# his0si/ConvNet-Quantization

Measured on AMD Instinct MI355X. Metric: images/sec at batch 1024 (3×32×32) int8 static-PTQ, 1/2/4/8 MI355X; top-1 delta, higher is better.
Workload: dtype int8; 1 GPU; full static-PTQ SimpleConvNet, all conv+linear int8 (u8 x s8 -> i32), NHWC, per-tensor weights; global_batch=1024, per_gpu_batch=1024, parallelism=dp1

## Files before the change

convnet-quantization_amd/csrc/conv3x3.hip:

```cpp
#include "common.hpp"
#include "conv_epi.hpp"
#include <type_traits>
#include <utility>
#include <algorithm>
#include <cmath>
#include "qconvnet_abi.hpp"

namespace qcn {

constexpr int kPipeD = 2;
constexpr int kSm56D = 4;
constexpr int kProdPrio = 2;

template <int CIN, int COUT, int HW, bool POOL, int WPX, int PSP = 16, int RPAD = 0,
          int SPAD = 0, bool SPLIT = false, int WI_ = 2, int JT_ = 4, int RB_ = 0>
struct ConvCfg {
  static constexpr int kCin = CIN, kCout = COUT;
  static constexpr bool kPool = POOL, kSplit = SPLIT;
  static constexpr int W = HW, H = HW;
  static constexpr int WI = WI_;
  static constexpr int JT = JT_;
  static constexpr int MPS = JT * WI;
  static constexpr int kWpx = WPX;
  static constexpr int WCO = COUT / (32 * WI);
// ... 1259 lines not shown
  static constexpr int OFF_CA = OFF_EB + 12 * CB::kCout;
  static constexpr int OFF_CB = OFF_CA + 4 * CA::kCout;
  static constexpr int LDS = OFF_CB + 4 * CB::kCout;
  static_assert(LDS <= 160 * 1024, "LDS budget");
  static constexpr int OPI = CB::OPX / SEGS;
};

template <class CA, class CB, int FA, int FB, bool KMAJOR, bool ILV = false>
QCN_DEV void convpair_ws16_body(int b, int G, const uint8_t* __restrict__ x, int nimg, int x_zp,
                                const int8_t* __restrict__ wa, const ConvEpi& epa, int xb_zp,
                                const int8_t* __restrict__ wb, const ConvEpi& epb, uint8_t* __restrict__ y) {
  using P = PairWs16<CA, CB>;
  using XA = Pix16<CA>;
  using XB = Pix16<CB>;
  constexpr int SEGS = P::SEGS, IMG = CA::IMG, W = CA::W, WCO = CA::WCO;
  constexpr int CH16 = CA::kCin / 16;
  extern __shared__ __attribute__((aligned(16))) uint8_t lds[];
  const int tid = threadIdx.x;
  const int role = __builtin_amdgcn_readfirstlane(tid >> 8);
  const int rt = tid & 255, lane = tid & 63, wave = rt >> 6;
  const int wc = wave % WCO, wp = wave / WCO;
  int T;
  if constexpr (ILV) {
    const int mine = b < nimg ? (nimg - 1 - b) / G + 1 : 0;
    T = (mine + SEGS - 1) / SEGS;
  } else {
    const int ntile = (nimg + SEGS - 1) / SEGS;
    T = b < ntile ? (ntile - 1 - b) / G + 1 : 0;
  }
  auto img_of = [&](int k, int sg) {
    const int n = ILV ? b + (k * SEGS + sg) * G : (b + k * G) * SEGS + sg;
    return n < nimg ? n : (ILV ? b + k * SEGS * G : (b + k * G) * SEGS);
  };
  auto in_src = [&](int k, int q) {
    const int p = rt + 256 * q;
    const int n = img_of(k, p / (IMG * CH16));
    return x + ((long)n * IMG + (p / CH16) % IMG) * CA::kCin + (p % CH16) * 16;
  };
  auto in_dst = [&](int q) {
    const int p = rt + 256 * q;
    const int pix = (p / CH16) % IMG;
    return CA::slot(p / (IMG * CH16), pix / W + 1, pix % W + 1) + (p % CH16) * 16;
  };
  uint4 sv0[4];
  if (role == 0 && T > 0) {
#pragma unroll
    for (int q = 0; q < 4; ++q) sv0[q] = *reinterpret_cast<const uint4*>(in_src(0, q));
  }
  float* eka = reinterpret_cast<float*>(lds + P::OFF_EA);
  float* ekb = reinterpret_cast<float*>(lds + P::OFF_EB);
  int* cra = reinterpret_cast<int*>(lds + P::OFF_CA);
  int* crb = reinterpret_cast<int*>(lds + P::OFF_CB);
  constexpr int NA = 3 * CA::kCout / 4, NB = 3 * CB::kCout / 4;
  constexpr int NCA = CA::kCout / 4, NCB = CB::kCout / 4;
  constexpr int NTAB = NA + NB + NCA + NCB, TPT = (NTAB + 255) / 256;
  float4 tval[TPT];
  auto tab = [&](int e, bool dst) -> float4* {
    if (e < NA) {
      const int a = e / (CA::kCout / 4), o = e % (CA::kCout / 4);
      const float* s = a == 0 ? epa.u : (a == 1 ? epa.v : epa.mult);
      return dst ? reinterpret_cast<float4*>(eka) + e : const_cast<float4*>(reinterpret_cast<const float4*>(s) + o);
    }
    e -= NA;
    if (e < NB) {
      const int a = e / (CB::kCout / 4), o = e % (CB::kCout / 4);
      const float* s = a == 0 ? epb.u : (a == 1 ? epb.v : epb.mult);
      return dst ? reinterpret_cast<float4*>(ekb) + e : const_cast<float4*>(reinterpret_cast<const float4*>(s) + o);
    }
    e -= NB;
    if (e < NCA)
      return dst ? reinterpret_cast<float4*>(cra) + e
                 : const_cast<float4*>(reinterpret_cast<const float4*>(epa.corr) + e);
    e -= NCA;
    return dst ? reinterpret_cast<float4*>(crb) + e
               : const_cast<float4*>(reinterpret_cast<const float4*>(epb.corr) + e);
  };
  {
    const uint32_t pa4 = xor80(splat_u8(x_zp)), pb4 = xor80(splat_u8(xb_zp));
    auto halo = [&](auto cfg, uint8_t* base, int nbuf, int pbytes, uint32_t pad) {
      using C = decltype(cfg);
      constexpr int HS = 2 * C::PCOLS + 2 * (C::PROWS - 2), CH = C::kCin / 16;
      const int total = nbuf * C::SEGS * HS * CH;
      for (int e = tid; e < total; e += 512) {
        const int c = e % CH, hs = (e / CH) % HS, sg = (e / (CH * HS)) % C::SEGS, bf = e / (CH * HS * C::SEGS);
        int pr, pc;
        if (hs < C::PCOLS) { pr = 0; pc = hs; }
        else if (hs < 2 * C::PCOLS) { pr = C::PROWS - 1; pc = hs - C::PCOLS; }
        else { const int r = hs - 2 * C::PCOLS; pr = 1 + (r >> 1); pc = (r & 1) ? C::PCOLS - 1 : 0; }
        *reinterpret_cast<uint4*>(base + bf * pbytes + C::slot(sg, pr, pc) + c * 16) = make_uint4(pad, pad, pad, pad);
      }
    };
    halo(CA{}, lds + P::OFF_PA, P::DOUBLE_A ? 2 : 1, P::PA, pa4);
    halo(CB{}, lds + P::OFF_PB, 2, P::PB, pb4);
  }
  if (role == 1) {
#pragma unroll
    for (int k = 0; k < TPT; ++k)
      if (rt + 256 * k < NTAB) tval[k] = *tab(rt + 256 * k, false);
#pragma unroll
    for (int k = 0; k < TPT; ++k)
      if (rt + 256 * k < NTAB) *tab(rt + 256 * k, true) = tval[k];
  }
  if (T == 0) return;

  const int p16 = lane & 15, g = lane >> 4;
  const wt_rsrc_t wra = wt_rsrc(wa), wrb = wt_rsrc(wb);
  const int voff = (wc * 64 + p16) * 64 + g * 16;
  auto pa_buf = [&](int j) { return lds + P::OFF_PA + (P::DOUBLE_A ? (j & 1) * P::PA : 0); };
  auto pb_buf = [&](int j) { return lds + P::OFF_PB + (j & 1) * P::PB; };
  auto write_in = [&](uint8_t* pa, const uint4 (&sv)[4]) {
#pragma unroll
    for (int q = 0; q < 4; ++q)
      *reinterpret_cast<uint4*>(pa + in_dst(q)) =
          make_uint4(xor80(sv[q].x), xor80(sv[q].y), xor80(sv[q].z), xor80(sv[q].w));
  };
  auto first_chunk = [&](wt_rsrc_t w0, v4i (&ga)[2][4]) {
#pragma unroll
    for (int i = 0; i < 4; ++i) {
      const auto v = __builtin_amdgcn_raw_buffer_load_b128(w0, voff, i * 1024, 0);
      ga[0][i] = (v4i){(int)v[0], (int)v[1], (int)v[2], (int)v[3]};
    }
  };

  v4i acc[4][8];
  if (role == 0) write_in(pa_buf(0), sv0);
  lds_barrier();

  struct Lane {
    int p16, g, ek;
    int la, lb;
    int hb;
    int q;
    const int *ca, *cb;
  };
  auto lanes = [&]() {
    int lz = lane;
    asm volatile("" : "+v"(lz));
    Lane L;
    L.p16 = lz & 15;
    L.g = lz >> 4;
    L.ek = wc * 64 + 4 * L.g;
    L.la = XA::at(wp, 0, L.p16) + 16 * L.g;
    L.lb = XB::at(wp, 0, L.p16) + 16 * L.g;
    L.hb = XA::template out_at<CB>(wp, 0, L.p16) + wc * 64 + 4 * L.g;
    L.q = wp * 32 + L.p16;
    L.ca = cra + (lz >> 6);
    L.cb = crb + (lz >> 6);
    return L;
  };
  auto epi_a = [&](const Lane& L, uint8_t* pb) {
    static_for<4>([&](auto ic) {
      constexpr int i = decltype(ic)::value;
      const EpiG K = load_epig(eka, CA::kCout, L.ek + 16 * i);
      static_for<8>([&](auto jc) {
        constexpr int j = decltype(jc)::value;
        uint32_t wd = 0;
#pragma unroll
        for (int r = 0; r < 4; ++r) wd = rq_elem<FA>(acc[i][j][r], K, r, epa, wd);
        *reinterpret_cast<uint32_t*>(pb + L.hb + XA::template out_jofs<CB>(j) + 16 * i) = xor80(wd);
      });
    });
  };
  auto epi_b = [&](const Lane& L, int k) {
    static_for<2>([&](auto gc) {
      constexpr int gq = decltype(gc)::value;
      uint32_t d[4];
      static_for<4>([&](auto ic) {
        constexpr int i = decltype(ic)::value;
        const EpiG K = load_epig(ekb, CB::kCout, L.ek + 16 * i);
        uint32_t wd = 0;
#pragma unroll
        for (int r = 0; r < 4; ++r) {
          const int a = max(max(acc[i][4 * gq][r], acc[i][4 * gq + 1][r]),
                            max(acc[i][4 * gq + 2][r], acc[i][4 * gq + 3][r]));
          wd = rq_elem<FB>(a, K, r, epb, wd);
        }
        d[i] = wd;
      });
      const auto s02 = __builtin_amdgcn_permlane32_swap(d[0], d[2], false, false);
      const auto s13 = __builtin_amdgcn_permlane32_swap(d[1], d[3], false, false);
      const auto t01 = __builtin_amdgcn_permlane16_swap(s02[0], s13[0], false, false);
      const auto t23 = __builtin_amdgcn_permlane16_swap(s02[1], s13[1], false, false);
      const uint4 v = make_uint4(t01[0], t01[1], t23[0], t23[1]);
      const int q = L.q + 16 * gq;
      const int n = img_of(k, q / P::OPI), pix = q % P::OPI;
      const int co = wc * 64 + 16 * L.g;
      const bool real = ILV ? b + (k * SEGS + q / P::OPI) * G < nimg : (b + k * G) * SEGS + q / P::OPI < nimg;
      if (real) {
        if constexpr (KMAJOR) {
          const int kc = (pix * CB::kCout + co) / 32;
          store_wt16(wt_rsrc(y), (uint32_t)(((long)kc * nimg + n) * 32 + 16 * (L.g & 1)), v);
        } else {
          store_wt16(wt_rsrc(y + (long)n * P::OPI * CB::kCout), (uint32_t)(pix * CB::kCout + co), v);
        }
      }
    });
  };

  if (role == 0) {
    v4i ga[2][4];
    first_chunk(wra, ga);
    uint4 sv[4] = {};
#pragma unroll 1
    for (int p = 0; p <= T; ++p) {
      if constexpr (!P::DOUBLE_A) {
        if (p >= 1 && p < T) write_in(pa_buf(p), sv);
        lds_barrier();
      }
      WS16_STAMP(p, 0);
      if (p < T) {
        const Lane L = lanes();
        pipe_job16<CA>(pa_buf(p), L.ca, wra, wra, voff, wc, L.la, L.g, acc, ga);
        WS16_STAMP(p, 1);
        const int kn = p + 1 < T ? p + 1 : p;
#pragma unroll
        for (int q = 0; q < 4; ++q) sv[q] = *reinterpret_cast<const uint4*>(in_src(kn, q));
        epi_a(L, pb_buf(p));
        if constexpr (P::DOUBLE_A) write_in(pa_buf(p + 1), sv);
        WS16_STAMP(p, 2);
      }
      lds_barrier();
    }
  } else {
    v4i ga[2][4];
    first_chunk(wrb, ga);
#pragma unroll 1
    for (int p = 0; p <= T; ++p) {
      if constexpr (!P::DOUBLE_A) lds_barrier();
      WS16_STAMP(p, 0);
      if (p >= 1) {
        const Lane L = lanes();
        if (p >= 2) epi_b(L, p - 2);
        WS16_STAMP(p, 1);
        pipe_job16<CB>(pb_buf(p - 1), L.cb, wrb, wrb, voff, wc, L.lb, L.g, acc, ga);
        WS16_STAMP(p, 2);
      }
      lds_barrier();
    }
    const Lane L = lanes();
    epi_b(L, T - 1);
#ifdef QCN_CONVNET_STAMP
    if (T + 1 < 8) { WS16_STAMP(T + 1, 0); }
#endif
  }
}

template <class CA, class CB, int FA, int FB, bool KMAJOR>
__global__ __launch_bounds__(512, 1)
void convpair_ws16_kernel(const uint8_t* __restrict__ x, int nimg, int x_zp, const int8_t* __restrict__ wa,
                          ConvEpi epa, int xb_zp, const int8_t* __restrict__ wb, ConvEpi epb,
                          uint8_t* __restrict__ y) {
  convpair_ws16_body<CA, CB, FA, FB, KMAJOR>((int)blockIdx.x, (int)gridDim.x, x, nimg, x_zp, wa, epa, xb_zp,
                                             wb, epb, y);
}

using W16A3 = ConvCfg<64, 128, 16, false, 2, 32, 0, 0, false>;
using W16B4 = ConvCfg<128, 128, 16, true, 2, 32, 64, 0, true>;
using W16A5 = ConvCfg<128, 256, 8, false, 1, 32, 192, 0, false>;
using W16B6 = ConvCfg<256, 256, 8, true, 1, 32, 0, 0, true>;

struct Conv1Cfg {
  static constexpr int H = 32, W = 32, R = 16, COUT = 64, NT = 256;
  static constexpr int PXB = R * W;
  static constexpr int PR = R + 2, PC = W + 2;
  static constexpr int PATCH = 3 * PR * PC;
  static constexpr int PATCH_AL = (PATCH + 15) / 16 * 16;
  static constexpr int KS = 32 + 16;
  static constexpr int LDS = PATCH_AL + PXB * KS;
};

template <int HW>
__global__ __launch_bounds__(256, 3)
void conv1_f32_kernel(const float* __restrict__ x, int nimg, float in_inv, int in_zp,
                      const int8_t* __restrict__ w1, ConvEpi ep, uint8_t* __restrict__ y,
                      uint8_t* __restrict__ qin_out) {
  constexpr int H = HW, W = HW;
  constexpr int R = (HW * HW >= 512) ? 512 / W : H;
  constexpr int SEGS = (HW * HW >= 512) ? 1 : 512 / (HW * HW);
  constexpr int PR = R + 2, PC = W + 2;
  constexpr int PATCH = SEGS * 3 * PR * PC;
  constexpr int PATCH_AL = (PATCH + 15) / 16 * 16;
  constexpr int KS = 48;
  extern __shared__ __attribute__((aligned(16))) uint8_t lds[];
  int8_t* patch = reinterpret_cast<int8_t*>(lds);
  uint8_t* cols = lds + PATCH_AL;

  const int tid = threadIdx.x, lane = tid & 63, wave = tid >> 6;
  const int l32 = lane & 31, hi = lane >> 5;
  const long p0 = (long)blockIdx.x * 512;
  const int n0 = (int)(p0 / (H * W));
  const int y0 = (int)((p0 % (H * W)) / W);
  const int8_t padv = (int8_t)(in_zp - 128);

  for (int it = tid; it < PATCH; it += 256) {
    const int seg = it / (3 * PR * PC);
    const int rem = it % (3 * PR * PC);
    const int c = rem / (PR * PC);
    const int rr = (rem / PC) % PR, cc = rem % PC;
    const int n = n0 + seg, yy = y0 + rr - 1, xx = cc - 1;
    int8_t v = padv;
    if (n < nimg && yy >= 0 && yy < H && xx >= 0 && xx < W) {
      const long gi = (((long)n * 3 + c) * H + yy) * W + xx;
      float t = x[gi] * in_inv;
      t = fminf(fmaxf(t, -1.0e9f), 1.0e9f);
      int q = (int)__builtin_rintf(t) + in_zp;
      q = q < 0 ? 0 : (q > 255 ? 255 : q);
      v = (int8_t)(q - 128);
      if (qin_out != nullptr && seg < SEGS && rr >= 1 && rr <= R && cc >= 1 && cc <= W)
        qin_out[(((long)n * H + yy) * W + xx) * 3 + c] = (uint8_t)q;
    }
    patch[it] = v;
  }
  __syncthreads();
  for (int pp = tid; pp < 512; pp += 256) {
    const int seg = pp / (R * W), yy = (pp / W) % R, xx = pp % W;
    uint32_t wds[8];
#pragma unroll
    for (int d = 0; d < 8; ++d) {
      uint32_t wv = 0;
#pragma unroll
      for (int bb = 0; bb < 4; ++bb) {
        const int k = d * 4 + bb;
        uint32_t byte = 0;
        if (k < 27) {
          const int tap = k / 3, c = k % 3, r = tap / 3, s = tap % 3;
          byte = (uint8_t)patch[((seg * 3 + c) * PR + yy + r) * PC + xx + s];
        }
        wv |= byte << (8 * bb);
      }
      wds[d] = wv;
    }
    uint4* dst = reinterpret_cast<uint4*>(cols + pp * KS);
    dst[0] = make_uint4(wds[0], wds[1], wds[2], wds[3]);
    dst[1] = make_uint4(wds[4], wds[5], wds[6], wds[7]);
  }
  __syncthreads();

  v4i a[2];
#pragma unroll
  for (int i = 0; i < 2; ++i)
    a[i] = *reinterpret_cast<const v4i*>(w1 + (i * 32 + l32) * 32 + hi * 16);
  v16i acc[2][4];
#pragma unroll
  for (int j = 0; j < 4; ++j) {
    const int m = (wave * 4 + j) * 32 + l32;
    const v4i b = *reinterpret_cast<const v4i*>(cols + m * KS + hi * 16);
#pragma unroll
    for (int i = 0; i < 2; ++i)
      acc[i][j] = __builtin_amdgcn_mfma_i32_32x32x32_i8(a[i], b, acc_init_corr(ep.corr, i * 32, hi),
                                                        0, 0, 0);
  }
  __syncthreads();
  uint8_t* lout = lds;
#pragma unroll
  for (int i = 0; i < 2; ++i)
#pragma unroll
    for (int j = 0; j < 4; ++j)
      epilogue_tile<1>(&acc[i][j], ep, i * 32, hi, lout + ((wave * 4 + j) * 32 + l32) * 80);
  __syncthreads();
  const long total = (long)nimg * H * W;
  store_staged<64, 80, 256>(lout, 512, y + p0 * 64, total - p0, tid);
}

using Conv2Cfg = ConvCfg<64, 64, 32, true, 4, 16, 96, 0, true>;

struct Conv12P {
  using C = Conv2Cfg;
  static constexpr int PATCH = C::PATCH;
  static constexpr int WRES = 9 * C::WBUF;
  static constexpr int IN_R = 20, IN_C = 40;
  static constexpr int IN8 = IN_R * IN_C * 4;
  static constexpr int OFF_W = 2 * PATCH;
  static constexpr int OFF_IN = OFF_W + WRES;
  static constexpr int OFF_EPI1 = OFF_IN + 2 * IN8;
  static constexpr int OFF_EPI2 = OFF_EPI1 + 12 * 64;
  static constexpr int OFF_CORR2 = OFF_EPI2 + 12 * 64;
  static constexpr int OFF_A1 = OFF_CORR2 + 4 * 64;
  static constexpr int OFF_CORR1 = OFF_A1 + 2 * 64 * 16;
  static constexpr int LDS = OFF_CORR1 + 4 * 64;
  static_assert(LDS <= 160 * 1024, "LDS budget");
  static constexpr int OFF_QLUT = LDS;
  static constexpr int LDS_U8 = OFF_QLUT + 3 * 256;
  static_assert(OFF_QLUT % 4 == 0 && LDS_U8 <= 160 * 1024, "LDS budget");
};

template <class C>
QCN_DEV void conv_mainloop_res(const uint8_t* patch, const uint8_t* wres,
                               const int* __restrict__ corr, int wave, int lane,
                               v16i (&acc)[2][4]) {
  constexpr int CB = C::kCin / 64;
  const int wc = wave % C::WCO, wp = wave / C::WCO;
  const int l32 = lane & 31, hi = lane >> 5;
  const PatchAddr<C> pa(wp, l32, hi);
  const int arow = wc * 64 + l32;
  const int aswz = (arow >> 2) & 3;
  v16i c0[2];
#pragma unroll
  for (int i = 0; i < 2; ++i) c0[i] = acc_init_corr(corr, wc * 64 + i * 32, hi);
  const uint8_t* abase = wres + arow * 64;
  auto rd_a = [&](int ch, int kk, int i) {
    return *reinterpret_cast<const v4i*>(abase + ch * C::WBUF + i * 32 * 64 +
                                         (((2 * kk + hi) ^ aswz) << 4));
  };
  auto rd_b = [&](int ch, int kk, int j) {
    const int tap = ch / CB, cb = ch % CB;
    return *reinterpret_cast<const v4i*>(patch + pa.base[j] + PatchAddr<C>::delta(tap, j) + cb * 64 +
                                         kk * 32);
  };
  auto step = [&](v4i (&fan)[2], v4i (&fbn)[4], int rch, int rkk, bool rd,
                  const v4i (&fa)[2], const v4i (&fb)[4], bool first) {
#pragma unroll
    for (int m = 0; m < 8; ++m) {
      if (rd) {
        if (m < 2) fan[m] = rd_a(rch, rkk, m);
        else if (m < 6) fbn[m - 2] = rd_b(rch, rkk, m - 2);
      }
      __builtin_amdgcn_sched_barrier(0);
      acc[m >> 2][m & 3] = __builtin_amdgcn_mfma_i32_32x32x32_i8(
          fa[m >> 2], fb[m & 3], first ? c0[m >> 2] : acc[m >> 2][m & 3], 0, 0, 0);
      __builtin_amdgcn_sched_barrier(0);
    }
  };
  v4i fa0[2], fb0[4], fa1[2], fb1[4];
  fa0[0] = rd_a(0, 0, 0);
  fa0[1] = rd_a(0, 0, 1);
#pragma unroll
  for (int j = 0; j < 4; ++j) fb0[j] = rd_b(0, 0, j);
#pragma unroll
  for (int ch = 0; ch < C::NCH; ++ch) {
    step(fa1, fb1, ch, 1, true, fa0, fb0, ch == 0);
    step(fa0, fb0, ch + 1, 0, ch + 1 < C::NCH, fa1, fb1, false);
  }
}

#ifdef QCN_C12_STAMP
__device__ unsigned long long g_c12_stamp[4096][3][12][3];
QCN_DEV void c12_stamp(int j, int k) {
  const unsigned long long t = __builtin_amdgcn_s_memtime();
  const unsigned lane = __builtin_amdgcn_mbcnt_hi(~0u, __builtin_amdgcn_mbcnt_lo(~0u, 0u));
  const int w = threadIdx.x >> 6;
  const int s = w == 0 ? 0 : (w == 4 ? 1 : (w == 5 ? 2 : -1));
  if (s >= 0 && lane == 0 && blockIdx.x < 4096 && j < 12) {
    volatile unsigned long long* d = &g_c12_stamp[blockIdx.x][s][j][k];
    *d = t + lane;
  }
}
#define C12_STAMP(j, k) c12_stamp(j, k)
#else
#define C12_STAMP(j, k)
#endif

template <class XT>
QCN_DEV void conv12p_body(int t0, int ts, int T, const XT* __restrict__ x, int nimg,
                          float in_inv, int in_zp, const int8_t* __restrict__ w1, ConvEpi ep1,
                          int x2_zp, const int8_t* __restrict__ w2, ConvEpi ep2,
                          uint8_t* __restrict__ y, const uint8_t* __restrict__ qlut = nullptr) {
  using C = Conv2Cfg;
  using L = Conv12P;
  constexpr bool U8 = std::is_same<XT, uint8_t>::value;
  static_assert(U8 || std::is_same<XT, float>::value, "fp32 NCHW or u8 NHWC input");
  extern __shared__ __attribute__((aligned(16))) uint8_t lds[];
  const int tid = threadIdx.x, lane = tid & 63, wave = tid >> 6;
  const bool producer = wave >= 4;
  const int ptid = tid - 320;
  auto tile_of = [&](int j) { return (t0 + (j >> 1) * ts) * 2 + (j & 1); };
  uint8_t* patch0 = lds;
  uint8_t* patch1 = lds + L::PATCH;
  uint8_t* in8_0 = lds + L::OFF_IN;
  uint8_t* in8_1 = lds + L::OFF_IN + L::IN8;

  typename std::conditional<U8, uint32_t, float4>::type xraw[3];
  const uint32_t padw = xor80(splat_u8(x2_zp));
  const uint4 pad4 = make_uint4(padw, padw, padw, padw);
  for (int e = tid; e < 2 * C::PROWS * 8; e += 512) {
    const int buf = e / (C::PROWS * 8), r = e % (C::PROWS * 8);
    const int pr = r / 8, pc = ((r / 4) & 1) ? C::PCOLS - 1 : 0, chunk = r & 3;
    *reinterpret_cast<uint4*>(lds + buf * L::PATCH + C::slot(0, pr, pc) + chunk * 16) = pad4;
  }

  auto setup = [&]() {
    if (!producer) {
      const int wave_u = __builtin_amdgcn_readfirstlane(wave);
#pragma unroll
      for (int i = 0; i < L::WRES / 4096; ++i) {
        const int p = i * 4 + wave_u;
        const int o = p * 1024 + lane * 16;
        const int ch = o / C::WBUF, oc = o % C::WBUF;
        const int r = oc >> 6, sl = (oc >> 4) & 3;
        glds16(w2 + (long)ch * C::WBUF + r * 64 + ((sl ^ ((r >> 2) & 3)) << 4), lds + L::OFF_W + p * 1024);
      }
    }

    const uint32_t in_pad = xor80(splat_u8(in_zp)) & 0x00ffffffu;
    for (int e = tid; e < 2 * L::IN_R * L::IN_C; e += 512) {
      const int b = e / (L::IN_R * L::IN_C), rc = e % (L::IN_R * L::IN_C);
      const int rr = rc / L::IN_C, cc = rc % L::IN_C;
      const bool pad_row = b == 0 ? rr < 2 : rr >= 18;
      if (pad_row || cc < 4 || cc >= 36)
        reinterpret_cast<uint32_t*>(lds + L::OFF_IN + b * L::IN8)[rc] = in_pad;
    }
    if (!producer) stage_epik<64, 256>(ep1, reinterpret_cast<float*>(lds + L::OFF_EPI1), tid);
    if (!producer) stage_epik<64, 256>(ep2, reinterpret_cast<float*>(lds + L::OFF_EPI2), tid);
    {
      int t = tid;
      asm volatile("" : "+v"(t));
      if (t < 16)
        reinterpret_cast<int4*>(lds + L::OFF_CORR2)[t] = reinterpret_cast<const int4*>(ep2.corr)[t];
      if (t >= 64 && t < 80)
        reinterpret_cast<int4*>(lds + L::OFF_CORR1)[t - 64] = reinterpret_cast<const int4*>(ep1.corr)[t - 64];
    }
    if (wave == 3) {
      const int l32 = lane & 31, hi = lane >> 5;
      v4i* a1t = reinterpret_cast<v4i*>(lds + L::OFF_A1);
#pragma unroll
      for (int i = 0; i < 2; ++i) {
        const uint4 r0 = *reinterpret_cast<const uint4*>(w1 + (i * 32 + l32) * 32);
        const uint4 r1 = *reinterpret_cast<const uint4*>(w1 + (i * 32 + l32) * 32 + 16);
        const uint32_t wd[8] = {r0.x, r0.y, r0.z, r0.w, r1.x, r1.y, r1.z, r1.w};
        auto byte = [&](int k) -> uint32_t { return (wd[k >> 2] >> (8 * (k & 3))) & 0xff; };
        auto tapw = [&](int t) -> int {
          return (int)(byte(3 * t) | (byte(3 * t + 1) << 8) | (byte(3 * t + 2) << 16));
        };
        const v4i lo4 = (v4i){tapw(0) | (int)(byte(24) << 24), tapw(1) | (int)(byte(25) << 24),
                              tapw(2) | (int)(byte(26) << 24), tapw(3)};
        const v4i hi4 = (v4i){tapw(4), tapw(5), tapw(6), tapw(7)};
        a1t[i * 64 + lane] = hi ? hi4 : lo4;
      }
    }
    if constexpr (U8) {
      for (int e = tid; e < 3 * 256; e += 512) lds[L::OFF_QLUT + e] = qlut[e] ^ 0x80;
    }
  };
  auto fresh_ptid = [&]() {
    int v = ptid;
    asm volatile("" : "+v"(v));
    return v;
  };
  auto stage_load = [&](int t) {
    if (ptid < 0) return;
    const int n = t >> 1, y0 = (t & 1) * 16;
    const int pt = fresh_ptid();
    const int r = pt < 144 ? pt >> 3 : 0, g = pt & 7;
    const int iy = y0 + (y0 == 0 ? 0 : -2) + r;
    const int nc = n < nimg ? n : nimg - 1;
    if constexpr (U8) {
      const uint32_t* p = reinterpret_cast<const uint32_t*>(x + (((long)nc * 32 + iy) * 32 + 4 * g) * 3);
#pragma unroll
      for (int c = 0; c < 3; ++c) xraw[c] = p[c];
    } else {
#pragma unroll
      for (int c = 0; c < 3; ++c)
        xraw[c] = *reinterpret_cast<const float4*>(x + (((long)nc * 3 + c) * 32 + iy) * 32 + 4 * g);
    }
  };
  auto stage_store = [&](uint8_t* in8, int half) {
    const int pt = fresh_ptid();
    if (pt >= 0 && pt < 144) {
      const int rr = (half ? 0 : 2) + (pt >> 3), g = pt & 7;
      uint32_t wd[4];
      if constexpr (U8) {
        const uint8_t* lut = lds + L::OFF_QLUT;
#pragma unroll
        for (int e = 0; e < 4; ++e) {
          uint32_t d = 0;
#pragma unroll
          for (int c = 0; c < 3; ++c) {
            const int k = 3 * e + c;
            const uint32_t b = (xraw[k >> 2] >> (8 * (k & 3))) & 0xffu;
            d |= (uint32_t)lut[c * 256 + b] << (8 * c);
          }
          wd[e] = d;
        }
      } else {
        const float zpf = (float)in_zp;
#pragma unroll
        for (int e = 0; e < 4; ++e) {
          uint32_t d = 0;
#pragma unroll
          for (int c = 0; c < 3; ++c) {
            const float xv = e == 0 ? xraw[c].x : e == 1 ? xraw[c].y : e == 2 ? xraw[c].z : xraw[c].w;
            d = __builtin_amdgcn_cvt_pk_u8_f32(__builtin_rintf(xv * in_inv) + zpf, c, d);
          }
          wd[e] = d ^ 0x00808080u;
        }
      }
      *reinterpret_cast<uint4*>(in8 + (rr * L::IN_C + 4 + 4 * g) * 4) = make_uint4(wd[0], wd[1], wd[2], wd[3]);
    }
  };
  auto fresh = [](int v) {
    asm volatile("" : "+v"(v));
    return v;
  };
  bool vuni = false, muni = false;
  const bool fast1 = epi_fast(ep1);
  auto conv1_tile = [&](int t, const uint8_t* in8, uint8_t* pb, const uint8_t* prev, int w,
                        int step) {
    __builtin_amdgcn_s_setprio(kProdPrio);
    const int h = t & 1, y0 = h * 16;
    const int r0 = h == 0 ? 1 : (prev ? 2 : 0), r1 = h == 0 ? 18 : 17;
    const int ln = fresh(lane), l32 = ln & 31, hi = ln >> 5;
    if (w == step - 1) {
      uint8_t* prow_ptr = pb + C::slot(0, h == 0 ? 0 : 17, l32 + 1);
      *reinterpret_cast<uint4*>(prow_ptr + hi * 32) = pad4;
      *reinterpret_cast<uint4*>(prow_ptr + hi * 32 + 16) = pad4;
    }
    if (prev) {
      for (int e = w * 64 + ln; e < 2 * C::RS / 16; e += step * 64)
        *reinterpret_cast<uint4*>(pb + C::slot(0, 0, 0) + e * 16) =
            *reinterpret_cast<const uint4*>(prev + C::slot(0, 16, 0) + e * 16);
    }
    const float* ek1 = reinterpret_cast<const float*>(lds + L::OFF_EPI1);
    v4i a1[2];
    v16i c1[2];
    {
      const v4i* a1t = reinterpret_cast<const v4i*>(lds + L::OFF_A1);
      const int* corr1 = reinterpret_cast<const int*>(lds + L::OFF_CORR1);
#pragma unroll
      for (int i = 0; i < 2; ++i) {
        a1[i] = a1t[i * 64 + ln];
        c1[i] = acc_init_corr(corr1, i * 32, hi);
      }
    }
    const int* in32 = reinterpret_cast<const int*>(in8);
    auto bop = [&](int tr, v4i& b0) {
      const int* r0 = in32 + (tr + 0) * L::IN_C + l32 + 3;
      const int* r1 = r0 + L::IN_C;
      const int* r2 = r1 + L::IN_C;
      if (hi == 0) {
        const uint32_t t8 = (uint32_t)r2[2];
        b0 = (v4i){(int)__builtin_amdgcn_perm((uint32_t)r0[0], t8, 0x00060504u),
                   (int)__builtin_amdgcn_perm((uint32_t)r0[1], t8, 0x01060504u),
                   (int)__builtin_amdgcn_perm((uint32_t)r0[2], t8, 0x02060504u), r1[0]};
      } else {
        b0 = (v4i){r1[1], r1[2], r2[0], r2[1]};
      }
    };
    auto rows = [&](auto mode) {
      constexpr int MODE = decltype(mode)::value > 2 ? decltype(mode)::value - 2 : decltype(mode)::value;
      constexpr bool AFF = decltype(mode)::value > 2;
      float u[2][16], m[2][16];
      const float sv = ek1[64], sm = ek1[128];
      if constexpr (MODE != 0) {
#pragma unroll
        for (int i = 0; i < 2; ++i)
#pragma unroll
          for (int g = 0; g < 4; ++g) {
            const int co = i * 32 + 8 * g + 4 * hi;
            const float4 u4 = *reinterpret_cast<const float4*>(ek1 + co);
            u[i][4 * g] = u4.x; u[i][4 * g + 1] = u4.y; u[i][4 * g + 2] = u4.z; u[i][4 * g + 3] = u4.w;
            if constexpr (MODE == 2) {
              const float4 m4 = *reinterpret_cast<const float4*>(ek1 + 128 + co);
              m[i][4 * g] = m4.x; m[i][4 * g + 1] = m4.y; m[i][4 * g + 2] = m4.z; m[i][4 * g + 3] = m4.w;
            }
          }
      }
      if constexpr (MODE == 0) {
        for (int tr = r0 + w; tr < r1; tr += step) {
          const int iy = y0 - 1 + tr;
          uint8_t* prow_ptr = pb + C::slot(0, tr, l32 + 1);
          if (iy < 0 || iy >= 32) {
            *reinterpret_cast<uint4*>(prow_ptr + hi * 32) = pad4;
            *reinterpret_cast<uint4*>(prow_ptr + hi * 32 + 16) = pad4;
            continue;
          }
          v4i b0;
          bop(tr, b0);
#pragma unroll
          for (int i = 0; i < 2; ++i) {
            v16i acc = __builtin_amdgcn_mfma_i32_32x32x32_i8(a1[i], b0, c1[i], 0, 0, 0);
            epilogue_tile_kf<1, true>(&acc, load_epik_lds(ek1, 64, i * 32, hi), ep1, i * 32, hi,
                                      prow_ptr);
          }
        }
      } else {
        const int wr = r0 + w;
        const int nr = (r1 - wr + step - 1) / step;
        auto mfma_row = [&](int tr, v16i (&acc)[2]) {
          v4i b0;
          bop(tr, b0);
#pragma unroll
          for (int i = 0; i < 2; ++i)
            acc[i] = __builtin_amdgcn_mfma_i32_32x32x32_i8(a1[i], b0, c1[i], 0, 0, 0);
        };
        auto requant_row = [&](const v16i (&acc)[2], int tr) {
          v2f t[2][8];
#pragma unroll
          for (int i = 0; i < 2; ++i)
#pragma unroll
            for (int e = 0; e < 16; ++e) {
              float f = (float)acc[i][e];
              f = __builtin_fmaf(u[i][e], sv, f);
              f = f * (MODE == 1 ? sm : m[i][e]);
              if constexpr (AFF) f = qdq_aff_f(f, ep1);
              t[i][e >> 1][e & 1] = f;
            }
          uint8_t* prow_ptr = pb + C::slot(0, tr, l32 + 1);
          uint32_t* pdw = reinterpret_cast<uint32_t*>(prow_ptr) + hi;
#pragma unroll
          for (int i = 0; i < 2; ++i)
#pragma unroll
            for (int g = 0; g < 4; ++g) {
              uint32_t wd = __builtin_amdgcn_cvt_pk_u8_f32(t[i][2 * g].x, 0, 0u);
              wd = __builtin_amdgcn_cvt_pk_u8_f32(t[i][2 * g].y, 1, wd);
              wd = __builtin_amdgcn_cvt_pk_u8_f32(t[i][2 * g + 1].x, 2, wd);
              wd = __builtin_amdgcn_cvt_pk_u8_f32(t[i][2 * g + 1].y, 3, wd);
              pdw[i * 8 + 2 * g] = xor80(wd);
            }
          const int iy = y0 - 1 + tr;
          if (iy < 0 || iy >= 32) {
            *reinterpret_cast<uint4*>(prow_ptr + hi * 32) = pad4;
            *reinterpret_cast<uint4*>(prow_ptr + hi * 32 + 16) = pad4;
          }
        };
        v16i acc_x[2], acc_y[2];
        if (nr > 0) mfma_row(wr, acc_x);
#pragma unroll
        for (int kr = 0; kr < 5; kr += 2) {
          if (kr >= nr) break;
          if (kr + 1 < nr) mfma_row(wr + step * (kr + 1), acc_y);
          requant_row(acc_x, wr + step * kr);
          if (kr + 1 < nr) {
            if (kr + 2 < nr) mfma_row(wr + step * (kr + 2), acc_x);
            requant_row(acc_y, wr + step * (kr + 1));
          }
        }
      }
    };
    if (fast1 && vuni) {
      if (muni) rows(std::integral_constant<int, 1>{});
      else rows(std::integral_constant<int, 2>{});
    } else if (ep1.qdq == 2 && vuni) {
      if (muni) rows(std::integral_constant<int, 3>{});
      else rows(std::integral_constant<int, 4>{});
    } else {
      rows(std::integral_constant<int, 0>{});
    }
  };
  auto conv2_tile = [&](int t, const uint8_t* pb) {
    const int ln = fresh(lane), l32 = ln & 31, hi = ln >> 5;
    v16i acc[2][4];
    conv_mainloop_res<C>(pb, lds + L::OFF_W, reinterpret_cast<const int*>(lds + L::OFF_CORR2),
                         wave, ln, acc);
    C12_STAMP(((t >> 1) - t0) / ts * 2 + (t & 1) + 1, 2);
    const int n = t >> 1, h = t & 1;
    const float* ek2 = reinterpret_cast<const float*>(lds + L::OFF_EPI2);
    uint8_t* dst = y + ((long)n * 256 + h * 128 + wave * 32 + l32) * 64;
    const uint8_t* wbase = y + ((long)n * 256 + h * 128) * 64;
    const uint32_t woff = (uint32_t)((wave * 32 + l32) * 64);
#pragma unroll
    for (int i = 0; i < 2; ++i)
      epilogue_tile_kf<4, false, false, true>(acc[i], load_epik_lds(ek2, 64, i * 32, hi), ep2, i * 32, hi,
                                              dst, wbase, woff);
  };

  if (producer && T > 0) stage_load(tile_of(0));
  setup();
  if constexpr (U8) __syncthreads();
  if (producer && T > 0) stage_store(in8_0, 0);
  if (!producer) asm volatile("s_waitcnt vmcnt(0)" ::: "memory");
  __syncthreads();
  {
    const float* ek1 = reinterpret_cast<const float*>(lds + L::OFF_EPI1);
    const int l = lane;
    vuni = __builtin_amdgcn_ballot_w64(ek1[64 + l] != ek1[64]) == 0;
    muni = __builtin_amdgcn_ballot_w64(ek1[128 + l] != ek1[128]) == 0;
  }
  constexpr bool SPLIT0 = true;
  for (int j = 0; j <= T; ++j) {
    C12_STAMP(j, 0);
    if (producer) {
      if (j + 1 < T) stage_load(tile_of(j + 1));
      if (j < T) {
        const bool split = SPLIT0 && j == 0;
        conv1_tile(tile_of(j), (j & 1) ? in8_1 : in8_0, (j & 1) ? patch1 : patch0,
                   (j & 1) ? patch0 : nullptr, split ? wave : wave - 4, split ? 8 : 4);
      }
      if (j + 1 < T) stage_store(((j + 1) & 1) ? in8_1 : in8_0, (j + 1) & 1);
    } else if (j >= 1) {
      conv2_tile(tile_of(j - 1), ((j - 1) & 1) ? patch1 : patch0);
    } else if (SPLIT0 && T > 0) {
      conv1_tile(tile_of(0), in8_0, patch0, nullptr, wave, 8);
      __builtin_amdgcn_s_setprio(0);
    }
    C12_STAMP(j, 1);
    __syncthreads();
  }
}

#ifndef QCN_CONV_U8_TU
__global__ __launch_bounds__(512, 1)
void conv12p_kernel(const float* __restrict__ x, int nimg, float in_inv, int in_zp,
                    const int8_t* __restrict__ w1, ConvEpi ep1, int x2_zp,
                    const int8_t* __restrict__ w2, ConvEpi ep2, uint8_t* __restrict__ y) {
  const int T = (int)blockIdx.x < nimg ? 2 * ((nimg - 1 - (int)blockIdx.x) / (int)gridDim.x + 1) : 0;
  conv12p_body((int)blockIdx.x, (int)gridDim.x, T, x, nimg, in_inv, in_zp, w1, ep1, x2_zp, w2, ep2, y);
}
#endif

#define QCN_C16_PARAMS                                                                                   \
  const int8_t* __restrict__ w0, ConvEpi e0, int z0, const int8_t* __restrict__ w1, ConvEpi e1, int z1, \
      const int8_t* __restrict__ w2, ConvEpi e2, int z2, const int8_t* __restrict__ w3, ConvEpi e3,      \
      int z3, const int8_t* __restrict__ w4, ConvEpi e4, int z4, const int8_t* __restrict__ w5,          \
      ConvEpi e5, int z5
#define QCN_C16_ARGS(L)                                                                                  \
  (L).w[0], (L).ep[0], (L).x_zp[0], (L).w[1], (L).ep[1], (L).x_zp[1], (L).w[2], (L).ep[2], (L).x_zp[2],   \
      (L).w[3], (L).ep[3], (L).x_zp[3], (L).w[4], (L).ep[4], (L).x_zp[4], (L).w[5], (L).ep[5], (L).x_zp[5]

struct ConvnetLayers {
  const int8_t* w[6];
  ConvEpi ep[6];
  int x_zp[6];
};

using SmA3 = ConvCfg<64, 128, 16, false, 4, 16, 96, 0, false, 2, 2>;
using SmB4 = ConvCfg<128, 128, 16, true, 2, 16, 32, 0, true, 1, 4>;
using SmA5 = ConvCfg<128, 256, 8, false, 1, 16, 224, 0, false, 1, 2>;
using SmB6 = ConvCfg<256, 256, 8, true, 1, 16, 32, 64, true, 1, 2>;

using WsA3 = ConvCfg<64, 128, 16, false, 2, 16, 96, 0, false>;
using WsB4 = ConvCfg<128, 128, 16, true, 2, 16, 32, 0, true>;
using WsA5 = ConvCfg<128, 256, 8, false, 1, 16, 224, 0, false>;
using WsB6 = ConvCfg<256, 256, 8, true, 1, 16, 32, 64, true>;

constexpr int cmax(int a, int b) { return a > b ? a : b; }
constexpr int kConvnet16Lds = cmax(Conv12P::LDS, cmax(PairWs16<W16A3, W16B4>::LDS, PairWs16<W16A5, W16B6>::LDS));
constexpr int kConvnetSmLds = cmax(Conv12P::LDS, cmax(PairCfg<SmA3, SmB4>::LDS, PairGaCfg<SmA5, SmB6>::LDS));

#ifdef QCN_CONVNET_STAMP
__device__ unsigned long long g_c16_stamp[4096][8];
QCN_DEV void c16_stamp(int i) {
  const unsigned long long t = __builtin_amdgcn_s_memtime();
  const unsigned long long r = __builtin_amdgcn_s_memrealtime();
  const unsigned lane = __builtin_amdgcn_mbcnt_hi(~0u, __builtin_amdgcn_mbcnt_lo(~0u, 0u));
  if ((threadIdx.x >> 6) == 0 && lane == 0 && blockIdx.x < 4096) {
    volatile unsigned long long* d = g_c16_stamp[blockIdx.x];
    d[i] = t + lane;
    d[4 + i] = r + lane;
  }
}
#define C16_STAMP(i) c16_stamp(i)
#else
#define C16_STAMP(i)
#endif

QCN_DEV void phase_boundary() {
  asm volatile("s_waitcnt vmcnt(0) lgkmcnt(0)" ::: "memory");
  __builtin_amdgcn_s_setprio(0);
  __syncthreads();
}

template <int EM, bool KMAJOR>
__global__ __launch_bounds__(512, 1)
void convnet_convs16_kernel(const float* __restrict__ x, int nimg, float in_inv, QCN_C16_PARAMS,
                            uint8_t* __restrict__ a2, uint8_t* __restrict__ a4, uint8_t* __restrict__ a6) {
  static_assert(PairWs16<W16A3, W16B4>::SEGS == 1, "conv3+4 tile k of workgroup b is image b + kG");
  const int b = (int)blockIdx.x, G = (int)gridDim.x;
  const int T = b < nimg ? 2 * ((nimg - 1 - b) / G + 1) : 0;
  C16_STAMP(0);
  conv12p_body(b, G, T, x, nimg, in_inv, z0, w0, e0, z1, w1, e1, a2);
  phase_boundary();
  C16_STAMP(1);
  convpair_ws16_body<W16A3, W16B4, EM, EM, false>(b, G, a2, nimg, z2, w2, e2, z3, w3, e3, a4);
  phase_boundary();
  C16_STAMP(2);
  convpair_ws16_body<W16A5, W16B6, EM, EM, KMAJOR, true>(b, G, a4, nimg, z4, w4, e4, z5, w5, e5, a6);
#ifdef QCN_CONVNET_STAMP
  __syncthreads();
#endif
  C16_STAMP(3);
}

#ifndef QCN_CONV_U8_TU
__global__ __launch_bounds__(512, 1)
void convnet_convs_sm_kernel(const float* __restrict__ x, int nimg, float in_inv, QCN_C16_PARAMS,
                             uint8_t* __restrict__ a2, uint8_t* __restrict__ a4, uint8_t* __restrict__ a6) {
  const int b = (int)blockIdx.x;
  C16_STAMP(0);
  conv12p_body(b, (int)gridDim.x, 2, x, nimg, in_inv, z0, w0, e0, z1, w1, e1, a2);
  phase_boundary();
  C16_STAMP(1);
  convpair_body<SmA3, SmB4>(b, a2, nimg, z2, w2, e2, z3, w3, e3, a4);
  phase_boundary();
  C16_STAMP(2);
  convpair_ga_body<SmA5, SmB6, kSm56D>(b, a4, nimg, z4, w4, e4, z5, w5, e5, a6);
#ifdef QCN_CONVNET_STAMP
  __syncthreads();
#endif
  C16_STAMP(3);
}
#endif

int convnet_convs_plan(int nimg, float in_scale, int in_zp, const qcn_conv_layer_t* layers, int kmajor,
                       ConvnetLayers& L, int& em, int& ncu);

#ifndef QCN_CONV_U8_TU
__global__ void conv3x3_generic_kernel(const uint8_t* __restrict__ x, int nimg, int H, int W,
                                       int cin, int x_zp, const int8_t* __restrict__ wpk,
                                       int tiled, int cout, ConvEpi ep, int pool,
                                       uint8_t* __restrict__ y) {
  const int OH = pool ? H / 2 : H, OW = pool ? W / 2 : W;
  const long total = (long)nimg * OH * OW * cout;
  for (long e = blockIdx.x * (long)blockDim.x + threadIdx.x; e < total;
       e += (long)gridDim.x * blockDim.x) {
    const int co = (int)(e % cout);
    const long pix = e / cout;
// ... 542 lines not shown
```

convnet-quantization_amd/csrc/conv_epi.hpp:

```cpp
#pragma once
#include "common.hpp"
#include "qconvnet_abi.hpp"
#include <utility>

namespace qcn {

struct ConvEpi {
  const float* u;
  const float* v;
  const float* mult;
  const int* corr;
  int zp_y, lo;
  int qdq;
  float s1; int z1; float inv2; int z2;
  int kmajor;
  float qa, qb, glo, ghi;
};

QCN_DEV float qdq_aff_f(float ab, const ConvEpi& ep) {
  return __builtin_amdgcn_fmed3f(__builtin_fmaf(__builtin_rintf(ab), ep.qa, ep.qb), ep.glo, ep.ghi);
}

__host__ __device__ inline bool epi_fast(const ConvEpi& ep) { return ep.zp_y == 0 && ep.lo == 0 && ep.qdq == 0; }
inline int epi_mode(const ConvEpi& ep) { return ep.qdq == 2 ? 2 : (epi_fast(ep) ? 1 : 0); }

void set_qdq(ConvEpi& ep, const qcn_qdq_t* q);

struct EpiG {
  float4 u, v, m;
};
QCN_DEV EpiG load_epig(const float* ek, int cout, int co) {
  return {*reinterpret_cast<const float4*>(ek + co), *reinterpret_cast<const float4*>(ek + cout + co),
          *reinterpret_cast<const float4*>(ek + 2 * cout + co)};
}
QCN_DEV float f4e(const float4& f, int e) { return e == 0 ? f.x : (e == 1 ? f.y : (e == 2 ? f.z : f.w)); }

template <class F, int... I>
QCN_DEV void static_for_impl(F&& f, std::integer_sequence<int, I...>) {
  (f(std::integral_constant<int, I>{}), ...);
}
template <int N, class F>
QCN_DEV void static_for(F&& f) {
  static_for_impl(f, std::make_integer_sequence<int, N>{});
}

template <int EM>
QCN_DEV uint32_t rq_elem(int a, const EpiG& K, int e, const ConvEpi& ep, uint32_t wd) {
  const float u = f4e(K.u, e), v = f4e(K.v, e), m = f4e(K.m, e);
  if constexpr (EM != 0) {
    float f = __builtin_fmaf(u, v, (float)a);
    f = f * m;
    if constexpr (EM == 2) f = qdq_aff_f(f, ep);
    return __builtin_amdgcn_cvt_pk_u8_f32(f, e, wd);
  } else {
    float q = requant_f(a, u, v, m, (float)ep.zp_y, (float)ep.lo);
    if (ep.qdq) q = qdq_next_f(q, ep.s1, (float)ep.z1, ep.inv2, (float)ep.z2);
    return __builtin_amdgcn_cvt_pk_u8_f32(q, e, wd);
  }
}

QCN_DEV void lds_barrier() {
  __builtin_amdgcn_sched_barrier(0);
  asm volatile("s_waitcnt lgkmcnt(0)" ::: "memory");
  __builtin_amdgcn_s_barrier();
  asm volatile("" ::: "memory");
  __builtin_amdgcn_sched_barrier(0);
}

}
```

Measured before the change: 8.168 million images/sec.

## Stage requant epilogues into fenced ILP batches and prefetch conv2 epilogue constants

Adds a staged requant helper that processes 8 or 16 accumulators one arithmetic step at a time, separated by scheduling barriers, so independent VALU ops sit back to back instead of forming dependent chains. The helper is used in the fused conv-A epilogue and the conv1 row requant. The conv2 epilogue now prefetches its first epilogue constants inside the last mainloop step through a new hook, and dispatches to a specialized epilogue mode chosen once per wave. The fences restrict compiler scheduling and hold more live registers, which could raise register pressure.

```diff
diff --git a/convnet-quantization_amd/csrc/conv3x3.hip b/convnet-quantization_amd/csrc/conv3x3.hip
--- a/convnet-quantization_amd/csrc/conv3x3.hip
+++ b/convnet-quantization_amd/csrc/conv3x3.hip
@@ -1435,13 +1435,30 @@
     static_for<4>([&](auto ic) {
       constexpr int i = decltype(ic)::value;
       const EpiG K = load_epig(eka, CA::kCout, L.ek + 16 * i);
-      static_for<8>([&](auto jc) {
-        constexpr int j = decltype(jc)::value;
-        uint32_t wd = 0;
-#pragma unroll
-        for (int r = 0; r < 4; ++r) wd = rq_elem<FA>(acc[i][j][r], K, r, epa, wd);
-        *reinterpret_cast<uint32_t*>(pb + L.hb + XA::template out_jofs<CB>(j) + 16 * i) = xor80(wd);
-      });
+      if constexpr (FA != 0) {
+        static_for<2>([&](auto jc) {
+          constexpr int j0 = 4 * decltype(jc)::value;
+          int a[16];
+#pragma unroll
+          for (int e = 0; e < 16; ++e) a[e] = acc[i][j0 + (e >> 2)][e & 3];
+          uint32_t wd[4];
+          rq_stages<FA, 16>(a, [&](int e) { return f4e(K.u, e & 3); }, [&](int e) { return f4e(K.v, e & 3); },
+                            [&](int e) { return f4e(K.m, e & 3); }, epa, wd);
+          static_for<4>([&](auto qc) {
+            constexpr int j = j0 + decltype(qc)::value;
+            *reinterpret_cast<uint32_t*>(pb + L.hb + XA::template out_jofs<CB>(j) + 16 * i) =
+                xor80(wd[decltype(qc)::value]);
+          });
+        });
+      } else {
+        static_for<8>([&](auto jc) {
+          constexpr int j = decltype(jc)::value;
+          uint32_t wd = 0;
+#pragma unroll
+          for (int r = 0; r < 4; ++r) wd = rq_elem<FA>(acc[i][j][r], K, r, epa, wd);
+          *reinterpret_cast<uint32_t*>(pb + L.hb + XA::template out_jofs<CB>(j) + 16 * i) = xor80(wd);
+        });
+      }
     });
   };
   auto epi_b = [&](const Lane& L, int k) {
@@ -1667,10 +1684,13 @@
   static_assert(OFF_QLUT % 4 == 0 && LDS_U8 <= 160 * 1024, "LDS budget");
 };
 
-template <class C>
+struct NoLate {
+  QCN_DEV void operator()() const {}
+};
+template <class C, class Late = NoLate>
 QCN_DEV void conv_mainloop_res(const uint8_t* patch, const uint8_t* wres,
                                const int* __restrict__ corr, int wave, int lane,
-                               v16i (&acc)[2][4]) {
+                               v16i (&acc)[2][4], Late&& late = Late{}) {
   constexpr int CB = C::kCin / 64;
   const int wc = wave % C::WCO, wp = wave / C::WCO;
   const int l32 = lane & 31, hi = lane >> 5;
@@ -1712,6 +1732,10 @@
 #pragma unroll
   for (int ch = 0; ch < C::NCH; ++ch) {
     step(fa1, fb1, ch, 1, true, fa0, fb0, ch == 0);
+    if (ch + 1 == C::NCH) {
+      late();
+      __builtin_amdgcn_sched_barrier(0);
+    }
     step(fa0, fb0, ch + 1, 0, ch + 1 < C::NCH, fa1, fb1, false);
   }
 }
@@ -1876,6 +1900,7 @@
   };
   bool vuni = false, muni = false;
   const bool fast1 = epi_fast(ep1);
+  const int mode2 = __builtin_amdgcn_readfirstlane(epi_fast(ep2) ? 1 : (ep2.qdq == 2 ? 2 : 0));
   auto conv1_tile = [&](int t, const uint8_t* in8, uint8_t* pb, const uint8_t* prev, int w,
                         int step) {
     __builtin_amdgcn_s_setprio(kProdPrio);
@@ -1966,29 +1991,19 @@
             acc[i] = __builtin_amdgcn_mfma_i32_32x32x32_i8(a1[i], b0, c1[i], 0, 0, 0);
         };
         auto requant_row = [&](const v16i (&acc)[2], int tr) {
-          v2f t[2][8];
-#pragma unroll
-          for (int i = 0; i < 2; ++i)
-#pragma unroll
-            for (int e = 0; e < 16; ++e) {
-              float f = (float)acc[i][e];
-              f = __builtin_fmaf(u[i][e], sv, f);
-              f = f * (MODE == 1 ? sm : m[i][e]);
-              if constexpr (AFF) f = qdq_aff_f(f, ep1);
-              t[i][e >> 1][e & 1] = f;
-            }
           uint8_t* prow_ptr = pb + C::slot(0, tr, l32 + 1);
           uint32_t* pdw = reinterpret_cast<uint32_t*>(prow_ptr) + hi;
 #pragma unroll
-          for (int i = 0; i < 2; ++i)
-#pragma unroll
-            for (int g = 0; g < 4; ++g) {
-              uint32_t wd = __builtin_amdgcn_cvt_pk_u8_f32(t[i][2 * g].x, 0, 0u);
-              wd = __builtin_amdgcn_cvt_pk_u8_f32(t[i][2 * g].y, 1, wd);
-              wd = __builtin_amdgcn_cvt_pk_u8_f32(t[i][2 * g + 1].x, 2, wd);
-              wd = __builtin_amdgcn_cvt_pk_u8_f32(t[i][2 * g + 1].y, 3, wd);
-              pdw[i * 8 + 2 * g] = xor80(wd);
-            }
+          for (int i = 0; i < 2; ++i) {
+            int a[16];
+#pragma unroll
+            for (int e = 0; e < 16; ++e) a[e] = acc[i][e];
+            uint32_t wd[4];
+            rq_stages<AFF ? 2 : 1, 16>(a, [&](int e) { return u[i][e]; }, [&](int) { return sv; },
+                                       [&](int e) { return MODE == 1 ? sm : m[i][e]; }, ep1, wd);
+#pragma unroll
+            for (int g = 0; g < 4; ++g) pdw[i * 8 + 2 * g] = xor80(wd[g]);
+          }
           const int iy = y0 - 1 + tr;
           if (iy < 0 || iy >= 32) {
             *reinterpret_cast<uint4*>(prow_ptr + hi * 32) = pad4;
@@ -2022,18 +2037,24 @@
   auto conv2_tile = [&](int t, const uint8_t* pb) {
     const int ln = fresh(lane), l32 = ln & 31, hi = ln >> 5;
     v16i acc[2][4];
+    const float* ek2 = reinterpret_cast<const float*>(lds + L::OFF_EPI2);
+    EpiK K0;
     conv_mainloop_res<C>(pb, lds + L::OFF_W, reinterpret_cast<const int*>(lds + L::OFF_CORR2),
-                         wave, ln, acc);
+                         wave, ln, acc, [&]() { K0 = load_epik_lds(ek2, 64, 0, hi); });
     C12_STAMP(((t >> 1) - t0) / ts * 2 + (t & 1) + 1, 2);
     const int n = t >> 1, h = t & 1;
-    const float* ek2 = reinterpret_cast<const float*>(lds + L::OFF_EPI2);
     uint8_t* dst = y + ((long)n * 256 + h * 128 + wave * 32 + l32) * 64;
     const uint8_t* wbase = y + ((long)n * 256 + h * 128) * 64;
     const uint32_t woff = (uint32_t)((wave * 32 + l32) * 64);
-#pragma unroll
-    for (int i = 0; i < 2; ++i)
-      epilogue_tile_kf<4, false, false, true>(acc[i], load_epik_lds(ek2, 64, i * 32, hi), ep2, i * 32, hi,
-                                              dst, wbase, woff);
+    auto epi2 = [&](auto em) {
+      constexpr int EM = decltype(em)::value;
+      epilogue_tile_k<4, false, EM, false, true>(acc[0], K0, ep2, 0, hi, dst, wbase, woff);
+      epilogue_tile_k<4, false, EM, false, true>(acc[1], load_epik_lds(ek2, 64, 32, hi), ep2, 32, hi, dst,
+                                                 wbase, woff);
+    };
+    if (mode2 == 1) epi2(std::integral_constant<int, 1>{});
+    else if (mode2 == 2) epi2(std::integral_constant<int, 2>{});
+    else epi2(std::integral_constant<int, 0>{});
   };
 
   if (producer && T > 0) stage_load(tile_of(0));
diff --git a/convnet-quantization_amd/csrc/conv_epi.hpp b/convnet-quantization_amd/csrc/conv_epi.hpp
--- a/convnet-quantization_amd/csrc/conv_epi.hpp
+++ b/convnet-quantization_amd/csrc/conv_epi.hpp
@@ -59,6 +59,44 @@
   }
 }
 
+QCN_DEV void rq_fence() { __builtin_amdgcn_sched_barrier(0); }
+template <int EM, int N, class KU, class KV, class KM>
+QCN_DEV void rq_stages(const int (&a)[N], KU&& ku, KV&& kv, KM&& km, const ConvEpi& ep,
+                       uint32_t (&wd)[N / 4]) {
+  static_assert(EM == 1 || EM == 2, "the general requant keeps its element-wise form");
+  static_assert(N == 8 || N == 16, "two or four destination dwords");
+  float c[N], f[N], g[N];
+  rq_fence();
+#pragma unroll
+  for (int i = 0; i < N; ++i) c[i] = (float)a[i];
+  rq_fence();
+#pragma unroll
+  for (int i = 0; i < N; ++i) f[i] = __builtin_fmaf(ku(i), kv(i), c[i]);
+  rq_fence();
+#pragma unroll
+  for (int i = 0; i < N; ++i) g[i] = f[i] * km(i);
+  rq_fence();
+  if constexpr (EM == 2) {
+    float r[N], h[N];
+#pragma unroll
+    for (int i = 0; i < N; ++i) r[i] = __builtin_rintf(g[i]);
+    rq_fence();
+#pragma unroll
+    for (int i = 0; i < N; ++i) h[i] = __builtin_fmaf(r[i], ep.qa, ep.qb);
+    rq_fence();
+#pragma unroll
+    for (int i = 0; i < N; ++i) g[i] = __builtin_amdgcn_fmed3f(h[i], ep.glo, ep.ghi);
+    rq_fence();
+  }
+#pragma unroll
+  for (int e = 0; e < 4; ++e) {
+#pragma unroll
+    for (int d = 0; d < N / 4; ++d)
+      wd[d] = __builtin_amdgcn_cvt_pk_u8_f32(g[4 * d + e], e, e == 0 ? 0u : wd[d]);
+    rq_fence();
+  }
+}
+
 QCN_DEV void lds_barrier() {
   __builtin_amdgcn_sched_barrier(0);
   asm volatile("s_waitcnt lgkmcnt(0)" ::: "memory");
```

Result: no change. 8.165 million images/sec, median of 2 (-0.0%).
